# facebookresearch/CODD

Hardware: AMD Instinct MI355X
Metric: frames/sec full CODD forward @960x540 (whole job) (higher is better)
Workload: dtype f32 (split-bf16 MFMA operands, f32 accumulate; HITNet + context network + Fusion exact f32); 1 GPU; full CODD (HITNetMF + Motion/RAFT3D iters=16 + Fusion) 960x540 padded to 960x576, max_disp=320, one video per GPU, steady-state frames (idx>=1), synthetic stereo sequence, random-init weights; conv_precision=split, hip_graph=True, frames_per_gpu=305, prewarm_frames=150, side_streams=True, library=codd_amd/csrc/libcodd_hip.so, full=False

## Files before the change

### codd_amd/_abi.py

```python
import ctypes as C
import os

from . import build as _build

c_float_p = C.POINTER(C.c_float)


class View(C.Structure):
    _fields_ = [("ptr", C.c_void_p), ("ctot", C.c_int), ("coff", C.c_int)]


class XsView(C.Structure):
    _fields_ = [("ptr", C.c_void_p), ("c8", C.c_int), ("hp", C.c_int), ("wp", C.c_int), ("bt", C.c_int),
                ("bl", C.c_int), ("o8", C.c_int), ("terms", C.c_int)]


class ConvParams(C.Structure):
    _fields_ = [
        ("in0", View), ("in1", View), ("C0", C.c_int), ("C1", C.c_int),
        ("B", C.c_int), ("Hin", C.c_int), ("Win", C.c_int),
        ("wpacked", C.c_void_p), ("bias", C.c_void_p),
        ("res1", View), ("res2", View), ("post", View),
        ("out", C.c_void_p), ("out_ctot", C.c_int), ("out_coff", C.c_int),
        ("Cout", C.c_int), ("Hout", C.c_int), ("Wout", C.c_int),
        ("kh", C.c_int), ("kw", C.c_int), ("sy", C.c_int), ("sx", C.c_int),
        ("pad_t", C.c_int), ("pad_l", C.c_int), ("dil_y", C.c_int), ("dil_x", C.c_int),
        ("act", C.c_int), ("store_mode", C.c_int), ("mb", C.c_int), ("npb", C.c_int), ("nw", C.c_int), ("ck", C.c_int), ("layout", C.c_int),
        ("terms", C.c_int), ("pgw", C.c_int), ("cgw", C.c_int),
        ("xs", C.c_void_p), ("xs_c8", C.c_int), ("xs_hp", C.c_int), ("xs_wp", C.c_int),
        ("xs_bt", C.c_int), ("xs_bl", C.c_int), ("xs_o8", C.c_int),
        ("xso", C.c_void_p), ("xso_c8", C.c_int), ("xso_hp", C.c_int), ("xso_wp", C.c_int), ("xso_bt", C.c_int),
        ("xso_bl", C.c_int), ("xso_o8", C.c_int), ("xso_terms", C.c_int), ("ksplit", C.c_int), ("dil2", C.c_int), ("gate", C.c_int),
    ]


ACT = dict(none=0, lrelu=1, relu=2, sigmoid=3, tanh=4, mish=5, relu_ch0=6)




class RollParams(C.Structure):
    _fields_ = [("in0", View), ("in1", View), ("C0", C.c_int), ("C1", C.c_int),
                ("B", C.c_int), ("H", C.c_int), ("W", C.c_int), ("C", C.c_int), ("mode", C.c_int),
                ("wA", C.c_void_p), ("bA", C.c_void_p), ("wB", C.c_void_p), ("bB", C.c_void_p),
                ("actA", C.c_int), ("actB", C.c_int), ("residual", C.c_int),
                ("out", C.c_void_p), ("out_ctot", C.c_int), ("out_coff", C.c_int), ("cout_store", C.c_int),
                ("rh", C.c_int)]


_i, _f, _p, _ll = C.c_int, C.c_float, C.c_void_p, C.c_longlong

SIGNATURES = {
    "codd_abi_version": (_i, []),
    "codd_conv2d": (_i, [C.POINTER(ConvParams), _p]),
    "codd_conv2d_check": (_i, [C.POINTER(ConvParams)]),
    "codd_conv2d_multi": (_i, [C.POINTER(ConvParams), _i, _p]),
    "codd_roll_packed_size": (_ll, [_i, _i, _i]),
    "codd_roll_pack_weights": (_i, [_p, _p, _i, _i, _i, _i, _p]),
    "codd_conv_roll": (_i, [C.POINTER(RollParams), _p]),
    "codd_conv2d_packed_size": (_ll, [_i] * 6),
    "codd_conv2d_pack_weights": (_i, [_p, _p, _i, _i, _i, _i, _i, _i, _p]),
    "codd_tile_costvol_argmin": (_i, [_p, _p, _i, _i, _i, _i, _i, _i, _p, _i, _i, _p, _i, _i, _i, _p]),
    "codd_tile_warp_cost": (_i, [_p, _p, _i, _i, _i, _i, View, View, _i, _p, _p, _p]),
    "codd_hyp_upsample": (_i, [View, _i, _i, _i, _f, _p, _i, _i, _p]),
    "codd_hyp_select": (_i, [_p, View, View, _i, _i, _i, _p, _i, _i, _p]),
    "codd_instnorm": (_i, [_p, _i, _i, _i, _p, _p, _i, _p, _p]),
    "codd_instnorm_xs": (_i, [_p, _i, _i, _i, _i, _p, _p, _i, _i, _p, XsView, _p]),
    "codd_conv2d_pack_weights_ex": (_i, [_p, _p, _i, _i, _i, _i, _i, _i, _ll, _ll, _f, _p]),
    "codd_allpairs_corr": (_i, [_p, _p, _i, _i, _i, _i, _p, _p, _p, _p, _p, _p]),
    "codd_allpairs_corr_scratch": (_ll, [_i, _i, _i, _i]),
    "codd_avgpool2": (_i, [_p, _i, _i, _i, _p, _p]),
    "codd_induced_flow": (_i, [_p, _p, _i, _i, _i, _f, _f, _f, _f, _p, _p]),
    "codd_context_split": (_i, [_p, _i, _i, _p, _p, _p]),
    "codd_se3_identity": (_i, [_p, _ll, _p]),
    "codd_corr_lookup": (_i, [_p, _p, _p, _p, _p, _i, _i, _i, _i, _p, _p]),
    "codd_raft_geometry": (_i, [_p, _p, _p, _i, _i, _i, _f, _f, _f, _f, _p, _p, _p]),
    "codd_se3_gn_step": (_i, [_p, _p, _i, _p, _p, _p, _p, _i, _i, _i, _f, _f, _f, _f, _i, _f, _f, _p, _p]),
    "codd_se3_gn_scratch": (_ll, [_i, _i, _i, _i]),
    "codd_set_option": (_i, [_i, _i]),
    "codd_get_option": (_i, [_i]),
    "codd_se3_gn_step_heads": (_i, [_p, XsView, _p, _p, _p, _p, _i, _i, _i, _f, _f, _f, _f, _i, _f, _f, _p, _p, _p]),
    "codd_cvx_upsample": (_i, [_p, _p, _i, _i, _i, _i, _i, _p, _p]),
    "codd_cvx_upsample_se3_weight": (_i, [_p, _p, _p, _i, _i, _i, _p, _p, _p]),
    "codd_disp_to_depth": (_i, [_p, _ll, _f, _p, _p]),
    "codd_subsample": (_i, [_p, _i, _i, _i, _i, _i, _i, _p, _p]),
    "codd_splat": (_i, [_p, _p, _i, _i, _i, _i, _i, _p, _i, _p, _i, _i, _i, _i, _i, _f, _f, _f, _f, _f, _f,
                        _p, _p, _p, _p]),
    "codd_splat_scratch": (_ll, [_i, _i, _i, _f]),
    "codd_resize_bilinear": (_i, [_p, _i, _i, _i, _i, _i, _i, _i, _p, _i, _i, _i, _i, _p]),
    "codd_resize_bilinear_add": (_i, [_p, _i, _i, _i, _i, _i, _i, _i, _p, _i, _i, _i, _i, _p, _p]),
    "codd_add_relu": (_i, [_p, _p, _ll, _i, _p, _p]),
    "codd_copy_many": (_i, [_p, _p, _p, _i, _p]),
    "codd_timestamp": (_i, [_p, _p]),
    "codd_gru_gate_zr": (_i, [_p, _p, _p, _p, _p, _p, _i, _i, _p, _p, _p]),
    "codd_gru_gate_q": (_i, [_p, _p, _p, _p, _p, _p, _p, _i, _i, _p, _p]),
    "codd_gru_gate_zr_xs": (_i, [_p, _p, _p, _p, _p, _p, _i, _i, _i, _p, XsView, _p]),
    "codd_gru_gate_q_xs": (_i, [_p, _p, _p, _p, _p, _p, _p, _i, _i, _i, _p, XsView, _p]),
    "codd_fusion_cues_lr": (_i, [_p] * 6 + [_i] * 7 + [_p, _p, _i, _i, _p]),
    "codd_fusion_cues_fr": (_i, [_p, _p, _p, _p, _i, _i, _i, _i, _p, _p]),
    "codd_fusion_forget": (_i, [_p, _p, _p, _p, _i, _i, _i, _i, _p, _p, _p]),
    "codd_disp_metrics": (_i, [_p, _p, _i, _i, _i, _i, _i, _f, _f, _f, _p, _p, _p]),
    "codd_raft_geometry_lookup": (_i, [_p, _p, _p, _p, _p, _p, _p, _i, _i, _i, _f, _f, _f, _f, _p, _p, _p, _p]),
    "codd_raft_geometry_lookup_xs": (_i, [_p, _p, _p, _p, _p, _p, _p, _i, _i, _i, _f, _f, _f, _f, _p, XsView, XsView, _p]),
    "codd_conv2d_packed_size_quad": (C.c_longlong, [_i, _i, _i, _i, _i, _i]),
    "codd_conv2d_pack_weights_quad": (_i, [_p, _p, _i, _i, _i, _i, _i, _i, _p]),
    "codd_split_bf16_bytes": (_ll, [_i] * 5),
    "codd_split_bf16": (_i, [View, _i, View, _i, _i, _i, _i, _i, _i, _i, _i, _i, _i, _p, _p]),
    "codd_conv2d_packed_bytes_bf16": (_ll, [_i] * 7),
    "codd_conv2d_pack_weights_bf16": (_i, [_p, _p, _i, _i, _i, _i, _i, _i, _i, _ll, _ll, _f, _p]),
    "codd_fusion_select": (_i, [_i, _p, _p, _p, _i, _i, _i, _i, _i, _f, _p, _p]),
    "codd_gt_motion": (_i, [_p, _p, _p, _i, _p, _p, _p, _i, _i, _i, _i, _i, _p, _p, _p, _p, _p, _p]),
    "codd_tepe_metrics": (_i, [_p, _p, _p, _p, _p, _p, _p, _i, _i, _i, _i, _i, _f, _f, _f, _p, _p, _p]),
    "codd_sceneflow_metrics": (_i, [_p] * 6 + [_i] * 5 + [_f] * 7 + [_p, _p, _p]),
    "codd_preprocess": (_i, [_p, _i, _i, _i, C.POINTER(C.c_float), C.POINTER(C.c_float), _i, _i, _p, _p]),
    "codd_fusion_blend": (_i, [_p, _p, _p, _p, _i, _i, _i, _i, _p, _p, _p, _p]),
    "codd_ingest_pair": (_i, [_p, _p, _i, _i, _i, c_float_p, c_float_p, _p, _p, _p, _p, _i, _i, _p, _p, _p]),
    "codd_export_depth": (_i, [_p, _i, _i, _i, _i, _i, _f, _p, _p]),
}

ABI_VERSION = 12
_lib = None
LOADED = None
MISSING = []
# ... 68 lines not shown
```

### codd_amd/motion.py

```python

import numpy as np
import torch
import torch.nn as nn

from . import ops
from .hrnet import ResizeConcatConv
from .ops import Slice
from .registry import MODELS, build_backbone, build_loss, register
from .stereo import cv, packed

BF_DEFAULT = 1050 * 0.2
MERGE_ENC_HEADS = True
FUSE_NORM_RECORDS = True
FUSE_GATES = True
FNET_CORESIDENT = False
PRELOOP_SIDE = True
ENC_CORESIDENT = 1
LOOP_FORK_ENC = True
LOOP_FORK_ZR = True

def packed_cat(mods):
    ver = tuple((m.weight.data_ptr(), m.weight._version, m.bias._version) for m in mods)
    cache = mods[0].__dict__.setdefault("_codd_packed_cat", {})
    key = tuple(id(m) for m in mods)
# ... 287 lines not shown
    row, kg = lane % 16, lane // 16
    k8 = torch.arange(8, device=dev)
    blocks = []
    for t in range(2):
        for s_ in range(8):
            cols = (32 * s_ + 8 * kg)[:, None] + k8[None]
            blocks.append(full[(16 * t + row)[:, None], cols])
    for s_ in range(16):
        cols = (256 + 32 * s_ + 8 * kg)[:, None] + k8[None]
        blocks.append(full[(32 + row)[:, None], cols])
    v = torch.stack(blocks, 0)
    if f16:
        hi = v.half()
        lo = (v - hi.float()).half()
        return torch.stack([hi, lo], 1).contiguous().view(torch.bfloat16)
    hi = v.bfloat16()
    lo = (v - hi.float()).bfloat16()
    return torch.stack([hi, lo], 1).contiguous()


@register
class RAFT3D(ops.RuntimeState, nn.Module):

    def __init__(self, cnet_cfg=None):
        super().__init__()
        self.hidden_dim = self.context_dim = 128
        self.corr_levels, self.corr_radius = 4, 3
        self.fnet = BasicEncoder(output_dim=128, norm_fn="instance")
        if cnet_cfg is None:
            raise NotImplementedError("the reference's FPN fallback is undefined upstream; pass cnet_cfg")
        cfg = dict(cnet_cfg)
        self.cnet = nn.Sequential(build_backbone(cfg),
                                  ResizeConcatConv(cfg["extra"]["stage4"]["num_channels"], 128 * 4))
        self.update_block = BasicUpdateBlock(hidden_dim=128)

    def context(self, image):
        with ops.stage("context"):
            return self.cnet[1](self.cnet[0](image))

    def prefetch(self, image, state=None):
        if ops.Fork.serial:
            self._pending = None
            return
        dev = image.device
        if getattr(self, "_side", None) is None or self._side[0].device != dev:
            self._side = (torch.cuda.Stream(device=dev), torch.cuda.Stream(device=dev))
        cur = torch.cuda.current_stream(dev)
        out = {}
        for key, stream, fn in (("fmap", self._side[0], self.fnet), ("netinp", self._side[1], self.context)):
            stream.wait_stream(cur)
            with torch.cuda.stream(stream):
                out[key] = fn(image)
                if key == "fmap" and state is not None and "memory" in state and state.get("raft_feat") is not None:
                    out["pyr"] = (state["raft_feat"], ops.allpairs_corr(state["raft_feat"], out["fmap"]))
                    if PRELOOP_SIDE and state.get("raft_netinp") is not None:
                        out["pre"] = self._preloop(state["raft_netinp"])
        self._pending = out

    def _preloop(self, net_inp):
        B, _, h, w = net_inp.shape
        ub = self.update_block
        net, inp = ops.context_split(net_inp)
        pre = dict(src=net_inp, net=net, inp=inp, T=ops.se3_identity(B, h, w, net_inp.device), zr=None)
        if ub._gates_fused(net) and ub.input_buffers(net)[0] is not None:
            ub._fused_now = True
            ub._h4(net), ub._ctx4(inp)
            fkz = ub._forks(net_inp.device)[1]
            prev, fkz.inline = fkz.inline, True
            try:
                pre["zr"] = ub.zr_convs(net)
            finally:
                fkz.inline = prev
        return pre

    def _join(self, key, dev):
        pend = getattr(self, "_pending", None)
        if not pend or key not in pend:
            return None
        if not getattr(self, "_nowait", False):
            torch.cuda.current_stream(dev).wait_stream(self._side[0] if key == "fmap" else self._side[1])
        return pend.pop(key)

    def forward(self, image_curr, depth_prev, depth_curr, intrinsics, state, outputs, iters=12, train_mode=False):
        dev = image_curr.device
        if "memory" not in state:
            fm, ni = self._join("fmap", dev), self._join("netinp", dev)
            state["raft_feat"] = fm if fm is not None else self.fnet(image_curr)
            state["raft_netinp"] = ni if ni is not None else self.context(image_curr)
            return
        B, _, H, W = image_curr.shape
        h, w = H // 8, W // 8
        K = [np.float32(v) for v in intrinsics]
        K8 = [float(v / np.float32(8.0)) for v in K]
        fmap_prev, net_inp = state["raft_feat"], state["raft_netinp"]
        pend = getattr(self, "_pending", None) or {}
        pl = pend.pop("pre", None)
        if pl is not None and pl["src"] is not net_inp:
            pl = None
        T = pl["T"] if pl is not None else ops.se3_identity(B, h, w, image_curr.device)
        pre = pend.pop("pyr", None)
        fmap_curr = self._join("fmap", dev)
        if fmap_curr is None:
            fmap_curr = self.fnet(image_curr)
        pyr = pre[1] if pre is not None and pre[0] is fmap_prev else ops.allpairs_corr(fmap_prev, fmap_curr)
        net, inp = (pl["net"], pl["inp"]) if pl is not None else ops.context_split(net_inp)
        if pl is not None and pl.get("depth_prev") is depth_prev:
            d1 = pl["d1"]
        else:
            d1 = ops.subsample(depth_prev.contiguous(), 3, 3, 8)
        d2 = ops.subsample(depth_curr.contiguous(), 3, 3, 8)
        mask = weight = None
        zr = pl["zr"] if pl is not None else None
        cxs, mxs = self.update_block.input_buffers(net)
        for it in range(iters):
            xyz, minfo, corr = ops.raft_geometry_lookup(T, d1, d2, K8, pyr, minfo_xs=mxs, corr_xs=cxs)
            net, mask, ae, delta, weight, zr, hid = self.update_block.run(
                net, inp, corr, minfo, need_mask=it == iters - 1, zr=zr, prefetch_next=it < iters - 1, fuse_heads=True)
            if hid is not None:
                weight = ops.se3_gn_step_heads(T, hid, *self.update_block.head_matrix(), xyz, d1, K8, radius=32)
            else:
                ops.se3_gn_step(T, ae, xyz, delta, weight, d1, K8, radius=32)
        self.update_block._forks(dev)[0].join()
        T_up, outputs["weight"] = ops.cvx_upsample_se3_weight(T, weight.contiguous(), mask)
        outputs["Ts"] = T_up
        outputs["flow2d_est_induced"] = ops.induced_flow(T_up, depth_prev, [float(v) for v in K])
        state["raft_feat"] = fmap_curr
        ni = self._join("netinp", dev)
        state["raft_netinp"] = ni if ni is not None else self.context(image_curr)


@register
class Motion(ops.RuntimeState, nn.Module):

    def __init__(self, raft3d=None, ds_scale=4, iters=16, loss=None):
        super().__init__()
        self.ds_scale = ds_scale
        self.iters = iters
        self.raft3d = MODELS.build(raft3d)
        self.loss = build_loss(loss) if loss is not None else None

    def prefetch(self, left_img, state=None, img_metas=None):
        self.raft3d.prefetch(left_img, state)
        pend = getattr(self.raft3d, "_pending", None)
        if PRELOOP_SIDE and pend and "pre" in pend and img_metas is not None and len(state.get("memory", ())) == 3:
            disp_prev = state["memory"][2]
            bf = self._bf(img_metas)
            with torch.cuda.stream(self.raft3d._side[0]):
                depth_prev = ops.disp_to_depth(disp_prev.contiguous(), bf)
                pend["pre"].update(disp_src=disp_prev, bf=bf, depth_prev=depth_prev,
                                   d1=ops.subsample(depth_prev.contiguous(), 3, 3, 8))

    @staticmethod
    def _bf(img_metas):
        fx = np.float32(img_metas[0]["intrinsics"][0])
        return float(np.float32(np.float32(BF_DEFAULT) / fx) * fx)

    def forward(self, state, outputs, img_metas, train_mode=False, **kwargs):
        img_curr = outputs["left_img"]
        if "memory" not in state:
            self.raft3d(img_curr, None, None, None, state, outputs, train_mode=train_mode)
            return
        intr = [np.float32(v) for v in img_metas[0]["intrinsics"]]
        bf = self._bf(img_metas)
        K = [float(v) for v in intr]
        img_prev, feat_prev, disp_prev = state["memory"]
        disp_curr = outputs["pred_disp"]
        pl = (getattr(self.raft3d, "_pending", None) or {}).get("pre")
        if pl is not None and pl.get("disp_src") is disp_prev and pl.get("bf") == bf:
            depth_prev = pl["depth_prev"]
        else:
            depth_prev = ops.disp_to_depth(disp_prev.contiguous(), bf)
        depth_curr = ops.disp_to_depth(disp_curr, bf).squeeze(1)
        self.raft3d(img_curr, depth_prev, depth_curr, intr, state, outputs, iters=self.iters, train_mode=train_mode)
        T_up = outputs["Ts"]
        B, H, W = depth_prev.shape
        ds, o = self.ds_scale, self.ds_scale // 2 - 1
        Kd = [float(v / np.float32(ds)) for v in intr]
        fk = self.__dict__.get("_fk")
        if fk is None or fk.dev != T_up.device:
# ... 7 lines not shown
```

### codd_amd/ops.py

```python
import collections
import ctypes as C

import torch

from . import _abi
from ._abi import ACT, ConvParams, View


class RuntimeState:
    _RUNTIME_KEYS = ("_side", "_pending", "_nowait", "_fk", "_xs", "_runners", "_kside", "_h4c", "_ctx4c", "_fused_now", "_pipe")

    def __getstate__(self):
        state = self.__dict__.copy()
        for k in self._RUNTIME_KEYS:
            state.pop(k, None)
        return state


class Slice:
    __slots__ = ("buf", "coff", "c")

    def __init__(self, buf, coff=0, c=None):
        assert buf.is_contiguous() and buf.dtype == torch.float32
        self.buf, self.coff = buf, coff
# ... 910 lines not shown
    _abi.check(lib.codd_tile_warp_cost(fl.data_ptr(), fr.data_ptr(), B, Cc, Ht, Wt, _view(hyp0), _view(hyp1),
                                       2 if hyp1 is not None else 1, out0.data_ptr(),
                                       None if out1 is None else out1.data_ptr(), _stream()), "tile_warp_cost")
    return out0, out1


def hyp_upsample(h, scale, out):
    lib = _abi.load()
    hs, os_ = _as_slice(h), _as_slice(out)
    B, _, hh, ww = hs.shape
    _abi.check(lib.codd_hyp_upsample(_view(hs), B, hh, ww, float(scale), os_.buf.data_ptr(), os_.buf.shape[1],
                                     os_.coff, _stream()), "hyp_upsample")
    return out


def hyp_select(upd, cur, prev, out):
    lib = _abi.load()
    B, _, hh, ww = upd.shape
    os_ = _as_slice(out)
    _abi.check(lib.codd_hyp_select(upd.data_ptr(), _view(cur), _view(prev), B, hh, ww, os_.buf.data_ptr(),
                                   os_.buf.shape[1], os_.coff, _stream()), "hyp_select")
    return out


def _f32(*shape, like):
    return torch.empty(*shape, device=like.device, dtype=torch.float32)


def instnorm(x, relu=True, res=None, res_relu=False, xs_out=None, want_fp32=True):
    lib = _abi.load()
    _require_gpu(x)
    B, Cc, H, W = x.shape
    stats = _f32(128 * B * Cc, like=x)
    if xs_out is not None:
        assert (xs_out.B, xs_out.H, xs_out.W) == (B, H, W) and Cc % 8 == 0 and Cc <= 8 * xs_out.c8
        y = torch.empty_like(x) if want_fp32 else None
        _abi.check(lib.codd_instnorm_xs(x.data_ptr(), B, Cc, H, W, stats.data_ptr(), _ptr(res), int(relu), int(res_relu),
                                        _ptr(y), _xs_view(xs_out), _stream()), "instnorm_xs")
        return y
    assert not res_relu
    y = torch.empty_like(x)
    _abi.check(lib.codd_instnorm(x.data_ptr(), B, Cc, H * W, stats.data_ptr(),
                                 None if res is None else res.data_ptr(), int(relu), y.data_ptr(), _stream()),
               "instnorm")
    return y


_ALLPAIRS_CFGS = ((2, 8, 32, 4, 2, 4, 2, 3, 1), (1, 16, 32, 4, 2, 4, 2, 3, 1), (1, 16, 32, 4, 2, 4, 1, 3, 1), (1, 12, 32, 4, 2, 4, 2, 3, 1),
                  (1, 12, 32, 4, 2, 4, 1, 3, 1), (1, 10, 32, 4, 2, 2, 2, 3, 1), (2, 8, 32, 4, 2, 4, 1, 3, 1),
                  (1, 8, 32, 2, 2, 4, 1, 3, 1), (1, 8, 16, 2, 2, 4, 1, 3, 1))
_ALLPAIRS_PICK = {}


def allpairs_corr_split(f1, f2):
    lib = _abi.load()
    _require_gpu(f1)
    B, D, h, w = f1.shape
    N = h * w
    lv = [_f32(B, N, (h >> i) * (w >> i), like=f1) for i in range(4)]
    srcs = [f2.contiguous()]
    for i in range(1, 4):
        hh, ww = h >> (i - 1), w >> (i - 1)
        nxt = _f32(B, D, hh >> 1, ww >> 1, like=f1)
        _abi.check(lib.codd_avgpool2(srcs[-1].data_ptr(), B * D, hh, ww, nxt.data_ptr(), _stream()), "avgpool2")
        srcs.append(nxt)
    packs = {}
    tune = _AUTOTUNE and not torch.cuda.is_current_stream_capturing()
    for i, src in enumerate(srcs):
        hh, ww = h >> i, w >> i
        p = ConvParams()
        p.C0, p.C1, p.B, p.Hin, p.Win, p.Cout, p.Hout, p.Wout = D, 0, 1, hh, ww, N, hh, ww
        p.kh = p.kw = p.sy = p.sx = p.dil_y = p.dil_x = 1
        p.terms, p.out_ctot = _split_terms(), N
        key = (D, hh, ww)
        cfg = _ALLPAIRS_PICK.get(key)
        if cfg is None:
            ok = [c for c in _ALLPAIRS_CFGS if _cfg_ok(lib, p, c)]
            if not ok:
                raise _abi.CoddHipError("all-pairs: no split-bf16 configuration for a %dx%d map" % (hh, ww))
            if any(decode_cfg(c).ck == 32 for c in ok):
                ok = [c for c in ok if decode_cfg(c).ck == 32]
            cfg = _allpairs_tune(lib, p, ok, f1[0], N, D) if tune else ok[0]
            if tune:
                _ALLPAIRS_PICK[key] = cfg
        f = decode_cfg(cfg)
        xs = _make_split(lib, p, src, None, [cfg], B=B)
        for b in range(B):
            if (f.mb, f.ck, b) not in packs:
                packs[(f.mb, f.ck, b)] = _pack_bf16(f1[b], N, D, 1, 1, f.mb, f.ck, p.terms, 1, N, 1.0 / 16.0)
            p.wpacked = packs[(f.mb, f.ck, b)].data_ptr()
            p.out = lv[i][b].data_ptr()
            p.xs = xs.buf.data_ptr() + b * (xs.buf.numel() // B)
            _set_cfg(p, cfg)
            _abi.check(_launch_conv(lib, p, _stream()), "allpairs conv")
    return lv


def _allpairs_tune(lib, p, cands, f1b, N, D):
    src = torch.zeros(1, D, p.Hin, p.Win, device=f1b.device)

    def apply(c):
        f = decode_cfg(c)
        xs = _make_split(lib, p, src, None, [c])
        wp = _pack_bf16(f1b, N, D, 1, 1, f.mb, f.ck, p.terms, 1, N, 1.0 / 16.0)
        p.wpacked = wp.data_ptr()
        _set_cfg(p, c)
        return xs, wp

    return _time_cfgs(lib, p, None, cands, apply, "allpairs %dx%d" % (p.Hin, p.Win))[0]


def allpairs_corr(f1, f2, split=None):
    if split is None:
        split = CONV_PRECISION in _SPLIT_MODES
    if split:
        return allpairs_corr_split(f1, f2)
    lib = _abi.load()
    _require_gpu(f1)
    B, D, h, w = f1.shape
    lv = [_f32(B, h * w, (h >> i) * (w >> i), like=f1) for i in range(4)]
    scratch = _f32(lib.codd_allpairs_corr_scratch(B, D, h, w), like=f1)
    _abi.check(lib.codd_allpairs_corr(f1.data_ptr(), f2.data_ptr(), B, D, h, w, lv[0].data_ptr(), lv[1].data_ptr(),
                                      lv[2].data_ptr(), lv[3].data_ptr(), scratch.data_ptr(), _stream()),
               "allpairs_corr")
    return lv


def corr_lookup(pyr, coords, h, w, out=None):
    lib = _abi.load()
    B = coords.shape[0]
    if out is None:
        out = _f32(B, 196, h, w, like=coords)
    _abi.check(lib.codd_corr_lookup(pyr[0].data_ptr(), pyr[1].data_ptr(), pyr[2].data_ptr(), pyr[3].data_ptr(),
                                    coords.data_ptr(), coords.shape[-1], B, h, w, out.data_ptr(), _stream()),
               "corr_lookup")
    return out


def raft_geometry(T, d1, d2, K8):
    lib = _abi.load()
    B, h, w, _ = T.shape
    xyz = _f32(B, h, w, 3, like=T)
    minfo = _f32(B, 9, h, w, like=T)
    _abi.check(lib.codd_raft_geometry(T.data_ptr(), d1.data_ptr(), d2.data_ptr(), B, h, w, *K8, xyz.data_ptr(),
                                      minfo.data_ptr(), _stream()), "raft_geometry")
    return xyz, minfo


def raft_geometry_lookup(T, d1, d2, K8, pyr, minfo_xs=None, corr_xs=None):
    lib = _abi.load()
    B, h, w, _ = T.shape
    if corr_xs is not None:
        xyz = _f32(B, h, w, 3, like=T)
        _abi.check(lib.codd_raft_geometry_lookup_xs(T.data_ptr(), d1.data_ptr(), d2.data_ptr(), pyr[0].data_ptr(),
                                                    pyr[1].data_ptr(), pyr[2].data_ptr(), pyr[3].data_ptr(), B, h, w,
                                                    *K8, xyz.data_ptr(), _xs_view(minfo_xs), _xs_view(corr_xs),
                                                    _stream()), "raft_geometry_lookup_xs")
        return xyz, None, None
    xyz, minfo, out = _f32(B, h, w, 3, like=T), _f32(B, 9, h, w, like=T), _f32(B, 196, h, w, like=T)
    _abi.check(lib.codd_raft_geometry_lookup(T.data_ptr(), d1.data_ptr(), d2.data_ptr(), pyr[0].data_ptr(),
                                             pyr[1].data_ptr(), pyr[2].data_ptr(), pyr[3].data_ptr(), B, h, w, *K8,
                                             xyz.data_ptr(), minfo.data_ptr(), out.data_ptr(), _stream()),
               "raft_geometry_lookup")
    return xyz, minfo, out


def se3_gn_step(T, ae, xyz, delta, weight, d1, K8, radius=32, lm=1e-4, ep=10.0):
    lib = _abi.load()
    B, h, w, _ = T.shape
# ... 419 lines not shown
```

### codd_amd/runtime.py

```python
import torch

from . import ops


class FrameRunner:

    def __init__(self, estimator, img_metas, use_graph=True, check_finite=False):
        self.est = estimator
        self.metas = img_metas
        self.use_graph = use_graph
        self.check_finite = check_finite
        self.last = {}
        self.state = {}
        self.graph = None
        self._static = None
        self.frames = 0

    def reset(self):
        self.state = {}
        self.frames = 0
        if self._static is not None:
            self._static["primed"] = False

    def _eager(self, left, right):
        out = self.est.consistent_online_depth_estimation(left, right, self.metas, self.state)
        self.last = {k: out[k] for k in ("Ts",) if out.get(k) is not None}
        return out["pred_disp"]

    def _state_tensors(self, state):
        mem = state["memory"]
        return [mem[0], mem[1], mem[2], state["raft_feat"], state["raft_netinp"]]

    def _capture(self, left, right):
        dev = left.device
        st = dict(l=torch.empty_like(left), r=torch.empty_like(right), primed=True)
        st["state"] = [torch.empty_like(t).contiguous() for t in self._state_tensors(self.state)]
        for dst, src in zip(st["state"], self._state_tensors(self.state)):
            dst.copy_(src)
        st["l"].copy_(left)
        st["r"].copy_(right)
        stream = torch.cuda.Stream(device=dev)
        stream.wait_stream(torch.cuda.current_stream(dev))
        g = torch.cuda.CUDAGraph()

        def body():
            s = st["state"]
            state = dict(memory=[s[0], s[1], s[2]], raft_feat=s[3], raft_netinp=s[4])
            out = self.est.consistent_online_depth_estimation(st["l"], st["r"], self.metas, state)
            ops.copy_many([(dst, src.contiguous()) for dst, src in zip(s, self._state_tensors(state))])
            st["last"] = {k: out[k] for k in ("Ts",) if out.get(k) is not None}
            return out["pred_disp"]

        saved = [t.clone() for t in st["state"]]
        with torch.cuda.stream(stream):
            body()
            for dst, src in zip(st["state"], saved):
                dst.copy_(src)
            torch.cuda.synchronize(dev)
            with torch.cuda.graph(g, stream=stream):
                st["out"] = body()
        torch.cuda.current_stream(dev).wait_stream(stream)
        for dst, src in zip(st["state"], saved):
            dst.copy_(src)
        self.graph, self._static = g, st

    def eager_frame_on_static_state(self, left, right):
        if self.est.motion is None and self.est.fusion is None:
            return self._eager(left, right)
        if self._static is not None and self._static.get("primed"):
            s = self._static["state"]
            state = dict(memory=[s[0], s[1], s[2]], raft_feat=s[3], raft_netinp=s[4])
        else:
            state = self.state
        out = self.est.consistent_online_depth_estimation(left, right, self.metas, state)
        if state is not self.state:
            for dst, src in zip(self._static["state"], self._state_tensors(state)):
                dst.copy_(src)
        return out["pred_disp"]

    def _capture_stateless(self, left, right):
        dev = left.device
        st = dict(l=left.clone(), r=right.clone(), primed=True, state=[])
        stream = torch.cuda.Stream(device=dev)
        stream.wait_stream(torch.cuda.current_stream(dev))
        g = torch.cuda.CUDAGraph()
        with torch.cuda.stream(stream):
            self._eager(st["l"], st["r"])
            torch.cuda.synchronize(dev)
            with torch.cuda.graph(g, stream=stream):
                st["out"] = self._eager(st["l"], st["r"])
        torch.cuda.current_stream(dev).wait_stream(stream)
        self.graph, self._static = g, st

    def step_fill(self, fill, scratch):
        st = self._static
        stateless = self.est.motion is None and self.est.fusion is None
        if not self.use_graph or self.graph is None or not (stateless or st["primed"]):
            fill(*scratch)
            return self.step(*scratch)
        self.frames += 1
        fill(st["l"], st["r"])
        self.graph.replay()
        if stateless:
            return st["out"]
        self.state = {"memory": True}
        self.last = st.get("last", {})
        if self.check_finite and not bool(torch.isfinite(st["out"]).all()):
            raise FloatingPointError(f"frame {self.frames}: non-finite disparity (conv precision {ops.CONV_PRECISION})")
        return st["out"]

    def step(self, left, right):
        self.frames += 1
        if self.use_graph and self.est.motion is None and self.est.fusion is None:
            if self.graph is None:
                self._capture_stateless(left, right)
            self._static["l"].copy_(left, non_blocking=True)
            self._static["r"].copy_(right, non_blocking=True)
            self.graph.replay()
            return self._static["out"]
        has_mem = "memory" in self.state or (self._static is not None and self._static.get("primed"))
        if not self.use_graph or not has_mem:
            d = self._eager(left, right)
            return d
        if self.graph is None:
# ... 15 lines not shown
```

### include/codd_hip.h

```cpp
#ifndef CODD_HIP_H
#define CODD_HIP_H

#ifdef __cplusplus
extern "C" {
#endif

#define CODD_ABI_VERSION 12

#define CODD_OK 0
#define CODD_EINVAL (-1)
#define CODD_EUNSUPPORTED (-2)

enum { CODD_OPT_GN_Q4 = 0, CODD_OPT_GN_BUILDER = 1, CODD_OPT_COUNT = 2 };
int codd_set_option(int key, int value);
int codd_get_option(int key);

enum { CODD_ACT_NONE = 0, CODD_ACT_LRELU02 = 1, CODD_ACT_RELU = 2, CODD_ACT_SIGMOID = 3,
       CODD_ACT_TANH = 4, CODD_ACT_MISH = 5, CODD_ACT_RELU_CH0 = 6 };

typedef struct {
  const float* ptr;
  int ctot;
  int coff;
} codd_view;
// ... 56 lines not shown
long long codd_conv2d_packed_bytes_bf16(int Cout, int Cin, int kh, int kw, int mb, int ck, int terms);
int codd_conv2d_pack_weights_bf16(const float* w, void* wpacked, int Cout, int Cin, int kh, int kw, int mb, int ck,
                                  int terms, long long co_stride, long long ci_stride, float scale, void* stream);

long long codd_conv2d_packed_size(int Cout, int Cin, int kh, int kw, int mb, int ck);
int codd_conv2d_pack_weights(const float* w, float* wpacked, int Cout, int Cin, int kh, int kw,
                             int mb, int ck, void* stream);
int codd_conv2d_pack_weights_ex(const float* w, float* wpacked, int Cout, int Cin, int kh, int kw,
                                int mb, int ck, long long co_stride, long long ci_stride, float scale,
                                void* stream);

typedef struct {
  codd_view in0, in1;
  int C0, C1;
  int B, H, W;
  int C;
  int mode;
  const float* wA;
  const float* bA;
  const float* wB;
  const float* bB;
  int actA, actB;
  int residual;
  float* out;
  int out_ctot, out_coff, cout_store;
  int rh;
} codd_roll_params;
long long codd_roll_packed_size(int C, int k, int Cin);
int codd_roll_pack_weights(const float* w, float* packed, int C, int Cout, int Cin, int k, void* stream);
int codd_conv_roll(const codd_roll_params* p, void* stream);

int codd_tile_costvol_argmin(const float* L, const float* R, int B, int C, int Ht, int Wt, int Wr, int D,
                             float* cost, int cost_ctot, int cost_coff,
                             float* disp, int disp_ctot, int disp_coff, int zero_dxdy, void* stream);

int codd_tile_warp_cost(const float* fl, const float* fr, int B, int C, int Ht, int Wt,
                        codd_view hyp0, codd_view hyp1, int nhyp,
                        float* out0, float* out1, void* stream);

int codd_hyp_upsample(codd_view in, int B, int h, int w, float scale,
                      float* out, int out_ctot, int out_coff, void* stream);

int codd_hyp_select(const float* upd, codd_view cur, codd_view prev, int B, int h, int w,
                    float* out, int out_ctot, int out_coff, void* stream);

int codd_instnorm(const float* x, int B, int C, int HW, float* stats, const float* res, int relu,
                  float* y, void* stream);
int codd_instnorm_xs(const float* x, int B, int C, int H, int W, float* stats, const float* res, int relu,
                     int relu_after_res, float* y, codd_xs_view xs, void* stream);

int codd_allpairs_corr(const float* f1, const float* f2, int B, int D, int h, int w,
                       float* lvl0, float* lvl1, float* lvl2, float* lvl3, float* scratch, void* stream);
long long codd_allpairs_corr_scratch(int B, int D, int h, int w);
int codd_avgpool2(const float* in, int BC, int h, int w, float* out, void* stream);

int codd_corr_lookup(const float* lvl0, const float* lvl1, const float* lvl2, const float* lvl3,
                     const float* coords, int cstride, int B, int h, int w, float* out, void* stream);

int codd_raft_geometry(const float* T, const float* depth1, const float* depth2, int B, int h, int w,
                       float fx, float fy, float cx, float cy, float* xyz, float* minfo, void* stream);

long long codd_se3_gn_scratch(int B, int h, int w, int radius);
int codd_se3_gn_step(float* T, const float* ae, int ae_c, const float* xyz, const float* delta,
                     const float* weight, const float* depth1, int B, int h, int w,
                     float fx, float fy, float cx, float cy, int radius, float lm, float ep,
                     float* Hb, void* stream);

int codd_se3_gn_step_heads(float* T, codd_xs_view hidden, const void* head_w, const float* head_b,
                           const float* xyz, const float* depth1, int B, int h, int w, float fx, float fy,
                           float cx, float cy, int radius, float lm, float ep, float* weight_out, float* Hb,
                           void* stream);

int codd_cvx_upsample(const float* data, const float* mask, int B, int h, int w, int dim, int mode,
                      float* out, void* stream);
int codd_cvx_upsample_se3_weight(const float* T, const float* weight, const float* mask, int B, int h, int w,
                                 float* T_out, float* weight_out, void* stream);

int codd_disp_to_depth(const float* disp, long long n, float bf, float* depth, void* stream);
int codd_subsample(const float* in, int B, int H, int W, int oy, int ox, int step, float* out, void* stream);

long long codd_splat_scratch(int B, int H, int W, float radius);
int codd_splat(const float* T, const float* depth, int HT, int WT, int oy, int ox, int ds,
               const float* featA, int CA, const float* featB, int CB, int with_flow,
               int B, int H, int W, float fx, float fy, float cx, float cy, float radius,
               float bf, float* out, float* zout, int* scratch, void* stream);

int codd_induced_flow(const float* T, const float* depth, int B, int H, int W,
                      float fx, float fy, float cx, float cy, float* out, void* stream);

int codd_context_split(const float* x, int B, int hw, float* net, float* inp, void* stream);

int codd_se3_identity(float* T, long long npix, void* stream);

int codd_resize_bilinear(const float* in, int B, int C, int Hi, int Wi, int Ho, int Wo, int align_corners,
                         float* out, int out_ctot, int out_coff, int accumulate, int relu, void* stream);
int codd_resize_bilinear_add(const float* in, int B, int C, int Hi, int Wi, int Ho, int Wo, int align_corners,
                             float* out, int out_ctot, int out_coff, int accumulate, int relu, const float* extra,
                             void* stream);

int codd_add_relu(const float* a, const float* b, long long n, int relu, float* y, void* stream);
int codd_copy_many(const float* const* src, float* const* dst, const long long* n, int count, void* stream);

int codd_timestamp(long long* slot, void* stream);

int codd_gru_gate_zr(const float* t1, const float* t2, const float* inp, const float* cor,
                     const float* mot, const float* h, int B, int hw, float* zr, float* rh, void* stream);
// ... 74 lines not shown
```

Measured before the change: 104.1 frames/s.

## Replace conv-based all-pairs correlation with split-bf16 MFMA GEMM and carried records

Result: slower. 102.6 frames/s (-1.4%).

```diff
diff --git a/codd_amd/_abi.py b/codd_amd/_abi.py
--- a/codd_amd/_abi.py
+++ b/codd_amd/_abi.py
@@ -69,6 +69,9 @@
     "codd_conv2d_pack_weights_ex": (_i, [_p, _p, _i, _i, _i, _i, _i, _i, _ll, _ll, _f, _p]),
     "codd_allpairs_corr": (_i, [_p, _p, _i, _i, _i, _i, _p, _p, _p, _p, _p, _p]),
     "codd_allpairs_corr_scratch": (_ll, [_i, _i, _i, _i]),
+    "codd_allpairs_records_bytes": (_ll, [_i, _i, _i, _i, _i]),
+    "codd_allpairs_records": (_i, [_p, _i, _i, _i, _i, _p, _p, _p]),
+    "codd_allpairs_gemm": (_i, [_p, _p, _i, _i, _i, _i, _p, _p, _p, _p, _p]),
     "codd_avgpool2": (_i, [_p, _i, _i, _i, _p, _p]),
     "codd_induced_flow": (_i, [_p, _p, _i, _i, _i, _f, _f, _f, _f, _p, _p]),
     "codd_context_split": (_i, [_p, _i, _i, _p, _p, _p]),
diff --git a/codd_amd/csrc/allpairs.hip b/codd_amd/csrc/allpairs.hip
--- /dev/null
+++ b/codd_amd/csrc/allpairs.hip
@@ -0,0 +1,253 @@
+#include "common.h"
+#include "codd_hip.h"
+#include <stdint.h>
+
+typedef __bf16 ap_bf16x8 __attribute__((ext_vector_type(8)));
+
+#define AP_TILE 128
+static inline int ap_np(int n) { return (n + AP_TILE - 1) / AP_TILE * AP_TILE; }
+
+struct ApGeom {
+  int B, D, h, w, N1, Np0;
+  int N2[4], Np[4];
+  int tiles_m, tiles_n[4];
+  int first[5];
+  long long poff[4];
+};
+
+static int ap_geometry(int B, int D, int h, int w, ApGeom& g) {
+  if (B < 1 || D < 1 || (h >> 3) < 1 || (w >> 3) < 1) return CODD_EINVAL;
+  if (D & 31) return CODD_EUNSUPPORTED;
+  g.B = B; g.D = D; g.h = h; g.w = w;
+  g.N1 = h * w; g.Np0 = ap_np(g.N1);
+  g.tiles_m = g.Np0 / AP_TILE;
+  long long off = 0, blocks = 0;
+  for (int i = 0; i < 4; ++i) {
+    g.N2[i] = (h >> i) * (w >> i);
+    g.Np[i] = ap_np(g.N2[i]);
+    g.tiles_n[i] = g.Np[i] / AP_TILE;
+    g.poff[i] = off;
+    off += (long long)B * 2 * (D / 8) * g.Np[i];
+    g.first[i] = (int)blocks;
+    blocks += (long long)B * g.tiles_m * g.tiles_n[i];
+    if (blocks > 0x7fffffffLL) return CODD_EUNSUPPORTED;
+  }
+  g.first[4] = (int)blocks;
+  return CODD_OK;
+}
+
+extern "C" long long codd_allpairs_records_bytes(int B, int D, int h, int w, int role) {
+  ApGeom g;
+  if (ap_geometry(B, D, h, w, g) != CODD_OK || role < 0 || role > 1) return -1;
+  if (role == 0) return (long long)B * 2 * (D / 8) * g.Np0 * 16;
+  return (g.poff[3] + (long long)B * 2 * (D / 8) * g.Np[3]) * 16;
+}
+
+template <int L>
+__device__ __forceinline__ float ap_pool(const float* __restrict__ c, int w, int y, int x) {
+  if constexpr (L == 0) {
+    return c[(size_t)y * w + x];
+  } else {
+    const float a = ap_pool<L - 1>(c, w, 2 * y, 2 * x), b = ap_pool<L - 1>(c, w, 2 * y, 2 * x + 1);
+    const float d = ap_pool<L - 1>(c, w, 2 * y + 1, 2 * x), e = ap_pool<L - 1>(c, w, 2 * y + 1, 2 * x + 1);
+    return (a + b + d + e) * 0.25f;
+  }
+}
+
+__device__ __forceinline__ void ap_put(uint4* __restrict__ dst, size_t plane, const float (&v)[8]) {
+  ap_bf16x8 hi, lo;
+#pragma unroll
+  for (int i = 0; i < 8; ++i) {
+    const __bf16 t = (__bf16)v[i];
+    hi[i] = t;
+    lo[i] = (__bf16)(v[i] - (float)t);
+  }
+  dst[0] = __builtin_bit_cast(uint4, hi);
+  dst[plane] = __builtin_bit_cast(uint4, lo);
+}
+
+__global__ __launch_bounds__(256) void allpairs_records_kernel(const float* __restrict__ f, ApGeom g, uint4* __restrict__ srec,
+                                                                uint4* __restrict__ prec, long long nrec, long long total) {
+  long long e = (long long)blockIdx.x * blockDim.x + threadIdx.x;
+  if (e >= total) return;
+  const int noct = g.D >> 3;
+  if (e >= nrec) {
+    e -= nrec;
+    int lvl = 2;
+    const long long per = (long long)g.B * g.D * g.N2[2];
+    if (e >= per) { e -= per; lvl = 3; }
+    const int n = g.N2[lvl], wl = g.w >> lvl;
+    const int pix = (int)(e % n);
+    const long long t = e / n;
+    const int ch = (int)(t % g.D), b = (int)(t / g.D);
+    const int y = pix / wl, x = pix - y * wl;
+    const float* c = f + ((size_t)b * g.D + ch) * (size_t)g.N1;
+    const float v = lvl == 2 ? ap_pool<2>(c, g.w, y, x) : ap_pool<3>(c, g.w, y, x);
+    const __bf16 hi = (__bf16)v, lo = (__bf16)(v - (float)hi);
+    const size_t plane = (size_t)noct * g.Np[lvl];
+    __bf16* dst = (__bf16*)(prec + g.poff[lvl] + ((size_t)b * 2 * noct + (ch >> 3)) * g.Np[lvl] + pix) + (ch & 7);
+    dst[0] = hi;
+    dst[plane * 8] = lo;
+    return;
+  }
+  int lvl = 0;
+  const long long per = (long long)g.B * noct * g.N2[0];
+  if (e >= per) { e -= per; lvl = 1; }
+  const int n = g.N2[lvl];
+  const int pix = (int)(e % n);
+  long long t = e / n;
+  const int oct = (int)(t % noct);
+  const int b = (int)(t / noct);
+  const int wl = g.w >> lvl;
+  const int y = pix / wl, x = pix - y * wl;
+  const float* c0 = f + ((size_t)b * g.D + oct * 8) * (size_t)g.N1;
+  float v[8];
+#pragma unroll
+  for (int i = 0; i < 8; ++i) {
+    const float* c = c0 + (size_t)i * g.N1;
+    v[i] = lvl == 0 ? ap_pool<0>(c, g.w, y, x) : ap_pool<1>(c, g.w, y, x);
+  }
+  if (prec) {
+    const size_t plane = (size_t)noct * g.Np[lvl];
+    ap_put(prec + g.poff[lvl] + ((size_t)b * 2 * noct + oct) * g.Np[lvl] + pix, plane, v);
+  }
+  if (lvl == 0 && srec) {
+#pragma unroll
+    for (int i = 0; i < 8; ++i) v[i] *= 1.0f / 16.0f;
+    const size_t plane = (size_t)noct * g.Np0;
+    ap_put(srec + ((size_t)b * 2 * noct + oct) * g.Np0 + pix, plane, v);
+  }
+}
+
+extern "C" int codd_allpairs_records(const float* f, int B, int D, int h, int w, void* srec, void* prec, void* stream) {
+  ApGeom g;
+  const int rc = ap_geometry(B, D, h, w, g);
+  if (rc != CODD_OK) return rc;
+  if (!f || (!srec && !prec) || ((uintptr_t)srec & 15) || ((uintptr_t)prec & 15)) return CODD_EINVAL;
+  const long long nrec = (long long)B * (D / 8) * (g.N2[0] + (prec ? g.N2[1] : 0));
+  const long long total = nrec + (prec ? (long long)B * D * (g.N2[2] + g.N2[3]) : 0);
+  allpairs_records_kernel<<<cdiv(total, 256), 256, 0, (hipStream_t)stream>>>(f, g, (uint4*)srec, (uint4*)prec, nrec, total);
+  CODD_LAUNCH_CHECK();
+  return CODD_OK;
+}
+
+struct ApOut { float* lv[4]; };
+
+constexpr int AP_ROW = 68;
+
+__global__ __launch_bounds__(256) void allpairs_gemm_kernel(const uint4* __restrict__ srec, const uint4* __restrict__ prec,
+                                                             const ApGeom g, const ApOut out) {
+  __shared__ __attribute__((aligned(16))) uint4 lds[2048];
+  const int tid = threadIdx.x, lane = tid & 63;
+  const int wave = __builtin_amdgcn_readfirstlane(tid >> 6);
+  const int j = lane & 15, gq = lane >> 4;
+  int bid = blockIdx.x, lvl = 0;
+  while (bid >= g.first[lvl + 1]) ++lvl;
+  bid -= g.first[lvl];
+  const int tn = bid % g.tiles_n[lvl]; bid /= g.tiles_n[lvl];
+  const int tm = bid % g.tiles_m;
+  const int b = bid / g.tiles_m;
+  const int noct = g.D >> 3, nch = g.D >> 5;
+  const int N2 = g.N2[lvl], Npl = g.Np[lvl];
+
+  const uint4* src[8];
+  const size_t step_s = (size_t)4 * g.Np0, step_p = (size_t)4 * Npl;
+#pragma unroll
+  for (int i = 0; i < 8; ++i) {
+    const int pl = (i >> 1) & 1, og = ((i & 1) << 1) | (tid >> 7), px = tid & 127;
+    if (i < 4) src[i] = srec + ((size_t)(b * 2 + pl) * noct + og) * g.Np0 + tm * AP_TILE + px;
+    else src[i] = prec + g.poff[lvl] + ((size_t)(b * 2 + pl) * noct + og) * Npl + tn * AP_TILE + px;
+  }
+  uint4 stage[8];
+#pragma unroll
+  for (int i = 0; i < 8; ++i) stage[i] = src[i][0];
+
+  const int wm = wave >> 1, wn = wave & 1;
+  f32x4 acc[4][4];
+#pragma unroll
+  for (int a = 0; a < 4; ++a)
+#pragma unroll
+    for (int m = 0; m < 4; ++m) acc[a][m] = (f32x4){0.f, 0.f, 0.f, 0.f};
+
+  const uint4* ls = lds + gq * 128 + wm * 64 + j;
+  const uint4* lp = lds + 1024 + gq * 128 + wn * 64 + j;
+  for (int ch = 0; ch < nch; ++ch) {
+    if (ch) __syncthreads();
+#pragma unroll
+    for (int i = 0; i < 8; ++i) lds[i * 256 + tid] = stage[i];
+    __syncthreads();
+    if (ch + 1 < nch) {
+#pragma unroll
+      for (int i = 0; i < 8; ++i) stage[i] = src[i][(size_t)(ch + 1) * (i < 4 ? step_s : step_p)];
+    }
+    ap_bf16x8 sh[4], sl[4], ph[4], pl[4];
+#pragma unroll
+    for (int m = 0; m < 4; ++m) {
+      sh[m] = __builtin_bit_cast(ap_bf16x8, ls[m * 16]);
+      sl[m] = __builtin_bit_cast(ap_bf16x8, ls[512 + m * 16]);
+    }
+#pragma unroll
+    for (int a = 0; a < 4; ++a) {
+      ph[a] = __builtin_bit_cast(ap_bf16x8, lp[a * 16]);
+      pl[a] = __builtin_bit_cast(ap_bf16x8, lp[512 + a * 16]);
+    }
+#pragma unroll
+    for (int a = 0; a < 4; ++a)
+#pragma unroll
+      for (int m = 0; m < 4; ++m) acc[a][m] = __builtin_amdgcn_mfma_f32_16x16x32_bf16(ph[a], sl[m], acc[a][m], 0, 0, 0);
+#pragma unroll
+    for (int a = 0; a < 4; ++a)
+#pragma unroll
+      for (int m = 0; m < 4; ++m) acc[a][m] = __builtin_amdgcn_mfma_f32_16x16x32_bf16(pl[a], sh[m], acc[a][m], 0, 0, 0);
+#pragma unroll
+    for (int a = 0; a < 4; ++a)
+#pragma unroll
+      for (int m = 0; m < 4; ++m) acc[a][m] = __builtin_amdgcn_mfma_f32_16x16x32_bf16(ph[a], sh[m], acc[a][m], 0, 0, 0);
+  }
+  __syncthreads();
+
+  float* strip = (float*)lds + wave * 2048;
+  float* o = out.lv[lvl] + (size_t)b * g.N1 * N2;
+  const int n1w = tm * AP_TILE + wm * 64, n2w = tn * AP_TILE + wn * 64;
+  const bool vec = (N2 & 3) == 0;
+#pragma unroll
+  for (int m = 0; m < 4; ++m) {
+#pragma unroll
+    for (int a = 0; a < 4; ++a) *(f32x4*)(strip + j * AP_ROW + 16 * a + 4 * gq) = acc[a][m];
+    __builtin_amdgcn_wave_barrier();
+    if (vec) {
+      const int col = n2w + 4 * j;
+#pragma unroll
+      for (int it = 0; it < 4; ++it) {
+        const int row = it * 4 + gq, n1 = n1w + 16 * m + row;
+        const f32x4 v = *(const f32x4*)(strip + row * AP_ROW + 4 * j);
+        if (n1 < g.N1 && col < N2) *(f32x4*)(o + (size_t)n1 * N2 + col) = v;
+      }
+    } else {
+      const int col = n2w + lane;
+#pragma unroll
+      for (int row = 0; row < 16; ++row) {
+        const int n1 = n1w + 16 * m + row;
+        const float v = strip[row * AP_ROW + lane];
+        if (n1 < g.N1 && col < N2) o[(size_t)n1 * N2 + col] = v;
+      }
+    }
+    __builtin_amdgcn_wave_barrier();
+  }
+}
+
+extern "C" int codd_allpairs_gemm(const void* srec, const void* prec, int B, int D, int h, int w, float* lvl0, float* lvl1,
+                                  float* lvl2, float* lvl3, void* stream) {
+  ApGeom g;
+  const int rc = ap_geometry(B, D, h, w, g);
+  if (rc != CODD_OK) return rc;
+  ApOut o = {{lvl0, lvl1, lvl2, lvl3}};
+  if (!srec || !prec || ((uintptr_t)srec & 15) || ((uintptr_t)prec & 15)) return CODD_EINVAL;
+  for (int i = 0; i < 4; ++i) {
+    if (!o.lv[i] || ((uintptr_t)o.lv[i] & 3)) return CODD_EINVAL;
+    if (!(g.N2[i] & 3) && ((uintptr_t)o.lv[i] & 15)) return CODD_EINVAL;
+  }
+  allpairs_gemm_kernel<<<g.first[4], 256, 0, (hipStream_t)stream>>>((const uint4*)srec, (const uint4*)prec, g, o);
+  CODD_LAUNCH_CHECK();
+  return CODD_OK;
+}
diff --git a/codd_amd/motion.py b/codd_amd/motion.py
--- a/codd_amd/motion.py
+++ b/codd_amd/motion.py
@@ -363,10 +363,13 @@
             with torch.cuda.stream(stream):
                 out[key] = fn(image)
                 if key == "fmap" and state is not None and "memory" in state and state.get("raft_feat") is not None:
-                    out["pyr"] = (state["raft_feat"], ops.allpairs_corr(state["raft_feat"], out["fmap"]))
+                    out["pyr"] = (state["raft_feat"],) + self._pyramid(state, state["raft_feat"], out["fmap"])
                     if PRELOOP_SIDE and state.get("raft_netinp") is not None:
                         out["pre"] = self._preloop(state["raft_netinp"])
         self._pending = out
+
+    def _pyramid(self, state, fmap_prev, fmap_curr):
+        return ops.allpairs_corr(fmap_prev, fmap_curr, prev=state.get("raft_rec"), carry=True, key=id(self))
 
     def _preloop(self, net_inp):
         B, _, h, w = net_inp.shape
@@ -397,6 +400,7 @@
         if "memory" not in state:
             fm, ni = self._join("fmap", dev), self._join("netinp", dev)
             state["raft_feat"] = fm if fm is not None else self.fnet(image_curr)
+            state.pop("raft_rec", None)
             state["raft_netinp"] = ni if ni is not None else self.context(image_curr)
             return
         B, _, H, W = image_curr.shape
@@ -413,7 +417,10 @@
         fmap_curr = self._join("fmap", dev)
         if fmap_curr is None:
             fmap_curr = self.fnet(image_curr)
-        pyr = pre[1] if pre is not None and pre[0] is fmap_prev else ops.allpairs_corr(fmap_prev, fmap_curr)
+        if pre is not None and pre[0] is fmap_prev:
+            pyr, rec = pre[1], pre[2]
+        else:
+            pyr, rec = self._pyramid(state, fmap_prev, fmap_curr)
         net, inp = (pl["net"], pl["inp"]) if pl is not None else ops.context_split(net_inp)
         if pl is not None and pl.get("depth_prev") is depth_prev:
             d1 = pl["d1"]
@@ -435,7 +442,7 @@
         T_up, outputs["weight"] = ops.cvx_upsample_se3_weight(T, weight.contiguous(), mask)
         outputs["Ts"] = T_up
         outputs["flow2d_est_induced"] = ops.induced_flow(T_up, depth_prev, [float(v) for v in K])
-        state["raft_feat"] = fmap_curr
+        state["raft_feat"], state["raft_rec"] = fmap_curr, rec
         ni = self._join("netinp", dev)
         state["raft_netinp"] = ni if ni is not None else self.context(image_curr)
 
diff --git a/codd_amd/ops.py b/codd_amd/ops.py
--- a/codd_amd/ops.py
+++ b/codd_amd/ops.py
@@ -986,7 +986,7 @@
 _ALLPAIRS_PICK = {}
 
 
-def allpairs_corr_split(f1, f2):
+def allpairs_corr_split_conv(f1, f2):
     lib = _abi.load()
     _require_gpu(f1)
     B, D, h, w = f1.shape
@@ -1044,11 +1044,71 @@
     return _time_cfgs(lib, p, None, cands, apply, "allpairs %dx%d" % (p.Hin, p.Win))[0]
 
 
-def allpairs_corr(f1, f2, split=None):
+_AP_BUFFERS = {}
+ALLPAIRS_GEMM = _os.environ.get("CODD_ALLPAIRS", "gemm") != "conv"
+
+
+def allpairs_records(f, key=None, source=True, pooled=True):
+    lib = _abi.load()
+    _require_gpu(f)
+    B, D, h, w = f.shape
+    f = f.contiguous()
+    srec = prec = None
+    if source:
+        srec = torch.empty(_abi_size(lib.codd_allpairs_records_bytes(B, D, h, w, 0)) // 4, device=f.device, dtype=torch.float32)
+    if pooled:
+        k = (key, B, D, h, w, str(f.device))
+        prec = _AP_BUFFERS.get(k)
+        if prec is None:
+            prec = _AP_BUFFERS[k] = torch.zeros(_abi_size(lib.codd_allpairs_records_bytes(B, D, h, w, 1)) // 4,
+                                                device=f.device, dtype=torch.float32)
+    _abi.check(lib.codd_allpairs_records(f.data_ptr(), B, D, h, w, _ptr(srec), _ptr(prec), _stream()), "allpairs_records")
+    return srec, prec
+
+
+def _abi_size(n):
+    if n <= 0:
+        raise _abi.CoddHipError("all-pairs records: unsupported feature-map shape (D %% 32 == 0, h, w >= 8)")
+    return n
+
+
+def allpairs_gemm(srec, prec, B, D, h, w):
+    lib = _abi.load()
+    lv = [_f32(B, h * w, (h >> i) * (w >> i), like=srec) for i in range(4)]
+    _abi.check(lib.codd_allpairs_gemm(srec.data_ptr(), prec.data_ptr(), B, D, h, w, lv[0].data_ptr(), lv[1].data_ptr(),
+                                      lv[2].data_ptr(), lv[3].data_ptr(), _stream()), "allpairs_gemm")
+    return lv
+
+
+def allpairs_corr_split(f1, f2, prev=None, key=None):
+    B, D, h, w = f1.shape
+    if prev is not None and prev[0] is f1 and prev[1] is not None:
+        s1 = prev[1]
+    else:
+        s1 = allpairs_records(f1, pooled=False)[0]
+    s2, p2 = allpairs_records(f2, key=key)
+    return allpairs_gemm(s1, p2, B, D, h, w), (f2, s2)
+
+
+def allpairs_carried(state):
+    if CONV_PRECISION != "split" or not ALLPAIRS_GEMM or state.get("raft_feat") is None:
+        return None
+    rec = state.get("raft_rec")
+    if rec is not None and rec[0] is state["raft_feat"] and rec[1] is not None:
+        return rec[1]
+    return allpairs_records(state["raft_feat"], pooled=False)[0]
+
+
+def allpairs_corr(f1, f2, split=None, prev=None, carry=False, key=None):
     if split is None:
         split = CONV_PRECISION in _SPLIT_MODES
+    if split and ALLPAIRS_GEMM and _split_terms() == 3 and f1.shape[1] % 32 == 0:
+        lv, nxt = allpairs_corr_split(f1, f2, prev, key)
+        return (lv, nxt) if carry else lv
+    if carry:
+        return allpairs_corr(f1, f2, split), None
     if split:
-        return allpairs_corr_split(f1, f2)
+        return allpairs_corr_split_conv(f1, f2)
     lib = _abi.load()
     _require_gpu(f1)
     B, D, h, w = f1.shape
diff --git a/codd_amd/runtime.py b/codd_amd/runtime.py
--- a/codd_amd/runtime.py
+++ b/codd_amd/runtime.py
@@ -29,7 +29,16 @@
 
     def _state_tensors(self, state):
         mem = state["memory"]
-        return [mem[0], mem[1], mem[2], state["raft_feat"], state["raft_netinp"]]
+        t = [mem[0], mem[1], mem[2], state["raft_feat"], state["raft_netinp"]]
+        rec = ops.allpairs_carried(state)
+        return t if rec is None else t + [rec]
+
+    @staticmethod
+    def _state_dict(s):
+        state = dict(memory=[s[0], s[1], s[2]], raft_feat=s[3], raft_netinp=s[4])
+        if len(s) > 5:
+            state["raft_rec"] = (s[3], s[5])
+        return state
 
     def _capture(self, left, right):
         dev = left.device
@@ -45,7 +54,7 @@
 
         def body():
             s = st["state"]
-            state = dict(memory=[s[0], s[1], s[2]], raft_feat=s[3], raft_netinp=s[4])
+            state = self._state_dict(s)
             out = self.est.consistent_online_depth_estimation(st["l"], st["r"], self.metas, state)
             ops.copy_many([(dst, src.contiguous()) for dst, src in zip(s, self._state_tensors(state))])
             st["last"] = {k: out[k] for k in ("Ts",) if out.get(k) is not None}
@@ -69,7 +78,7 @@
             return self._eager(left, right)
         if self._static is not None and self._static.get("primed"):
             s = self._static["state"]
-            state = dict(memory=[s[0], s[1], s[2]], raft_feat=s[3], raft_netinp=s[4])
+            state = self._state_dict(s)
         else:
             state = self.state
         out = self.est.consistent_online_depth_estimation(left, right, self.metas, state)
diff --git a/include/codd_hip.h b/include/codd_hip.h
--- a/include/codd_hip.h
+++ b/include/codd_hip.h
@@ -132,6 +132,10 @@
 int codd_allpairs_corr(const float* f1, const float* f2, int B, int D, int h, int w,
                        float* lvl0, float* lvl1, float* lvl2, float* lvl3, float* scratch, void* stream);
 long long codd_allpairs_corr_scratch(int B, int D, int h, int w);
+long long codd_allpairs_records_bytes(int B, int D, int h, int w, int role);
+int codd_allpairs_records(const float* f, int B, int D, int h, int w, void* srec, void* prec, void* stream);
+int codd_allpairs_gemm(const void* srec, const void* prec, int B, int D, int h, int w, float* lvl0, float* lvl1,
+                       float* lvl2, float* lvl3, void* stream);
 int codd_avgpool2(const float* in, int BC, int h, int w, float* out, void* stream);
 
 int codd_corr_lookup(const float* lvl0, const float* lvl1, const float* lvl2, const float* lvl3,
```
